# cfframe/spatial-VAE

Measured on AMD Instinct MI355X. Metric: images/sec (ELBO fwd+bwd+step), MNIST 28x28 batch=256, 1/2/4/8 GPU, higher is better.
Workload: dtype f32; 1 GPU; mnist-rotated-translated 28x28 z=2 H=500x2 tanh B=256 (BASELINE configs[1]); global_batch=256, per_gpu_batch=256, pixels=784, parallelism=dp1

## Files before the change

spatial_vae_amd/csrc/api.hip:

```cpp
#include <stdarg.h>
#include <stdio.h>
#include <stdlib.h>
#include <string.h>
#include <math.h>
#include <atomic>
#include <mutex>
#include <iterator>
#include <type_traits>
#include <unordered_map>
#include <vector>

#include "common.h"
#include <hip/hip_ext.h>
#include "dense.h"
#include "wgrad2.h"
#include "elementwise.h"
#include "encoder.h"
#include "split.h"

using namespace svae;

namespace {

thread_local char g_err[512] = "";
// ... 79 lines not shown
    return on;
}

bool split_a0_fragments_only(const Geo& g) {
    static const bool on = [] { const char* e = getenv("SVAE_SPLIT_A0"); return e && e[0] == '1'; }();
    const char* fuse = getenv("SVAE_FUSE_OUT");
    return on && split_mode() && split_l0_on() && split_wgrad_on() && !(fuse && fuse[0] == '1') &&
           (g.act == SVAE_ACT_TANH || g.act == SVAE_ACT_SIGMOID) && g.ntile % 2 == 0 && g.L == 2 && g.in_dim == 2 &&
           !(g.flags & SVAE_FLAG_RESID);
}

int fuse_out_mode() {
    const char* e = getenv("SVAE_FUSE_OUT");
    if (!e) return 2;
    return e[0] == '0' ? 0 : (e[0] == '1' ? 1 : 2);
}
bool split_active(const Geo& g) {
    return split_mode() && (g.act == SVAE_ACT_TANH || g.act == SVAE_ACT_SIGMOID) && g.ntile % 2 == 0;
}
bool rank1_out(const Geo& g) {
    return fuse_out_mode() == 2 && !split_active(g) && g.C == 1 && g.L >= 2 && !(g.flags & SVAE_FLAG_RESID) &&
           (g.act == SVAE_ACT_TANH || g.act == SVAE_ACT_SIGMOID);
}

struct PlanBits {
    unsigned bits;
    unsigned long long seq;
};
std::mutex g_plan_mu;
std::unordered_map<const void*, PlanBits> g_plans;
unsigned long long g_plan_seq = 0;
unsigned plan_bits(const Geo& g) {
    return (rank1_out(g) ? 1u : 0u) | (split_active(g) ? 2u : 0u) | ((unsigned)fuse_out_mode() << 2) |
           (split_a0_fragments_only(g) ? 16u : 0u) | ((split_mode() && split_l0_on()) ? 32u : 0u);
}
void remember_plan(const void* saved, unsigned bits) {
    std::lock_guard<std::mutex> lk(g_plan_mu);
    if (g_plans.size() >= 4096) {
        const unsigned long long cut = g_plan_seq - 2048;
        for (auto it = g_plans.begin(); it != g_plans.end();) it = it->second.seq < cut ? g_plans.erase(it) : std::next(it);
    }
    g_plans[saved] = PlanBits{bits, g_plan_seq++};
}
long recorded_plan(const void* saved) {
    std::lock_guard<std::mutex> lk(g_plan_mu);
    auto it = g_plans.find(saved);
    return it == g_plans.end() ? -1L : (long)it->second.bits;
}

constexpr int kFinishMaxChunks = 64;
int finish_chunks(int N) {
    int c = (N + 1023) / 1024;
    return c < 1 ? 1 : (c > kFinishMaxChunks ? kFinishMaxChunks : c);
}

Plan make_plan(const Geo& g, void* saved, void* ws) {
    Plan p;
    const size_t MH = (size_t)g.Mp * g.Hp;
    Carver cs(saved);
    for (int l = 0; l < g.L; ++l) p.act[l] = cs.take<float>(MH);
    p.savedC = split_mode() ? cs.take<uint4>(MH / 4) : nullptr;
    float* swf[SVAE_MAX_HIDDEN];
    float* swb[SVAE_MAX_HIDDEN];
    for (int l = 0; l + 1 < g.L; ++l) {
        swf[l] = cs.take<float>((size_t)g.Hp * g.Hp);
        swb[l] = cs.take<float>((size_t)g.Hp * g.Hp);
    }
// ... 90 lines not shown
    if ((long)d->B * ((d->N + 31) / 32 * 32) > (1L << 30)) return fail(SVAE_E_INVALID, "B*N too large");
    return SVAE_OK;
}

int check_params(const svae_desc* d, const svae_params* p) {
    if (!p || !p->coord_w || !p->coord_b || !p->out_w || !p->out_b) return fail(SVAE_E_INVALID, "missing parameter pointer");
    if (d->Zd > 0 && !p->latent_w) return fail(SVAE_E_INVALID, "latent_dim > 0 but latent_w is null");
    if ((d->flags & SVAE_FLAG_BILINEAR) && !p->bilinear_w) return fail(SVAE_E_INVALID, "bilinear flag but bilinear_w is null");
    for (int l = 0; l + 1 < d->L; ++l)
        if (!p->hidden_w[l] || !p->hidden_b[l]) return fail(SVAE_E_INVALID, "hidden layer %d parameters are null", l);
    return SVAE_OK;
}

int check_pose(const svae_pose* pose) {
    if (!pose) return fail(SVAE_E_INVALID, "null pose");
    if (!pose->coords && !pose->grid) return fail(SVAE_E_INVALID, "pose needs coords or grid");
    return SVAE_OK;
}

int check_ws(const Plan& p, const void* ws, size_t ws_bytes) {
    if (!ws) return fail(SVAE_E_WORKSPACE, "null workspace");
    if (reinterpret_cast<uintptr_t>(ws) & 255) return fail(SVAE_E_WORKSPACE, "workspace not 256-byte aligned");
    if (ws_bytes < p.ws_bytes) return fail(SVAE_E_WORKSPACE, "workspace too small: %zu < %zu", ws_bytes, p.ws_bytes);
    return SVAE_OK;
}

enum Kind { K_PREPARE = 0, K_LAYER0_FWD, K_DENSE_FWD, K_OUT_FWD, K_DLOGITS, K_OUT_BWD, K_WGRAD, K_WGRAD_REDUCE,
            K_DENSE_DGRAD, K_LAYER0_BWD, K_SMALL_BWD, K_BCE, K_GAUSSIAN, K_LATENT, K_ADAM, K_AUGMENT, K_ENCODER, K_COUNT };
const char* const kKindNames[SVAE_PROF_KINDS] = {"prepare", "layer0_fwd", "dense_fwd", "out_fwd", "dlogits", "out_bwd",
                                                 "wgrad", "wgrad_reduce", "dense_dgrad", "layer0_bwd", "small_bwd", "bce",
                                                 "gaussian", "latent", "adam", "augment", "encoder", "", "", ""};
static_assert(K_COUNT <= SVAE_PROF_KINDS, "svae_profile_read arrays too small");
enum Path { P_DENSE_FP32_FWD = 0, P_DENSE_FP32_DGRAD, P_WGRAD_FP32, P_DENSE_SPLIT_FWD, P_DENSE_SPLIT_DGRAD, P_WGRAD_SPLIT,
            P_OUT_BWD_STREAM, P_OUT_BWD_SPLIT, P_OUT_BWD_RANK1, P_OUT_BWD_FUSED_GENERIC, P_DENSE4, P_DENSE4_TAIL, P_WGRAD2, P_COUNT };
const char* const kPathNames[SVAE_PATH_KINDS] = {"dense_fp32_fwd", "dense_fp32_dgrad", "wgrad_fp32", "dense_split_fwd",
                                                  "dense_split_dgrad", "wgrad_split", "out_bwd_stream", "out_bwd_split",
                                                  "out_bwd_rank1", "out_bwd_fused_generic", "dense4", "dense4_tail", "wgrad2", "", "", ""};
static_assert(P_COUNT <= SVAE_PATH_KINDS, "svae_path_counts array too small");
std::atomic<long long> g_path[SVAE_PATH_KINDS];
inline void took(int path) { g_path[path].fetch_add(1, std::memory_order_relaxed); }

struct ProfRec { hipEvent_t a, b; int kind; };
int g_prof_level = 0;
std::vector<ProfRec> g_prof_used, g_prof_free;

struct Scope;
thread_local Scope* t_attach = nullptr;

struct Scope {
    hipStream_t st;
    ProfRec rec;
    bool on, attach, carried;
    Scope(int kind, hipStream_t s, bool attach_to_launch = false) : st(s), on(false), attach(attach_to_launch), carried(false) {
        std::lock_guard<std::mutex> lk(g_prof_mu);
        if (g_prof_level == 0) return;
        if (g_prof_level == 1 && kind != K_DENSE_FWD && kind != K_DENSE_DGRAD && kind != K_WGRAD) return;
        if (!g_prof_free.empty()) {
            rec = g_prof_free.back();
            g_prof_free.pop_back();
        } else if (hipEventCreate(&rec.a) != hipSuccess || hipEventCreate(&rec.b) != hipSuccess) {
            return;
        }
        rec.kind = kind;
        on = true;
        if (attach) t_attach = this;
        else (void)hipEventRecord(rec.a, st);
    }
    ~Scope() {
        if (!on) return;
        if (attach) t_attach = nullptr;
// ... 253 lines not shown
        if (!cols_ready)
            hipLaunchKernelGGL(split_cols_kernel, dim3(blocks_for(g.noct * g.Hp)), dim3(256), 0, st, dh, pl.splitC[0], g.noct,
                               g.Hp, (const float*)pl.gscale);
        if (!aprev_cols)
            hipLaunchKernelGGL(split_cols_kernel, dim3(blocks_for(g.noct * g.Hp)), dim3(256), 0, st, aprev, pl.splitC[1],
                               g.noct, g.Hp, (const float*)nullptr);
    }
    Scope prof(K_WGRAD, st);
    static bool attr_set = false;
    if (!attr_set) {
        (void)hipFuncSetAttribute(reinterpret_cast<const void*>(&split_wgrad_kernel<true>),
                                  hipFuncAttributeMaxDynamicSharedMemorySize, kSplitWgradLds);
        (void)hipFuncSetAttribute(reinterpret_cast<const void*>(&split_wgrad_kernel<false>),
                                  hipFuncAttributeMaxDynamicSharedMemorySize, kSplitWgradLds);
        attr_set = true;
    }
    SplitWgradArgs w;
    w.dh = pl.splitC[0]; w.ap = aprev_cols ? aprev_cols : pl.splitC[1]; w.slab = pl.slab; w.bslab = pl.bslab; w.gscale = pl.gscale;
    w.nsteps = (long)g.Mp / 16; w.Hp = g.Hp; w.nblk1 = pl.wg_nblk1; w.S = pl.wg_S;
    const dim3 grid(pl.wg_nblk1 * pl.wg_nblk1 * pl.wg_S);
    if (cols_ready) hipLaunchKernelGGL(split_wgrad_kernel<false>, grid, dim3(256), kSplitWgradLds, st, w);
    else hipLaunchKernelGGL(split_wgrad_kernel<true>, grid, dim3(256), kSplitWgradLds, st, w);
}

int use_dense4(const Geo& g, int resid, int lastd) {
    const char* e = getenv("SVAE_DENSE4");
    const int mode = e ? (e[0] == '0' ? 0 : (e[0] == '2' ? 2 : 1)) : 3;
    if (mode == 0 || g.tiles % 4 != 0 || resid || lastd == 1) return 0;
    const bool nt2_ok = g.ntile % 2 == 0;
    if (mode == 2) return nt2_ok ? 2 : 1;
    if (mode == 1) return 1;
    const long wgs2 = ((g.tiles / 4 + 3) / 4) * (g.ntile / 2);
    return (nt2_ok && wgs2 >= 2048) ? 2 : 1;
}

template <int NT, bool DGRAD, bool FIRST, int LASTD, int CF>
void launch_dense4_v(const DenseArgs& a, long groups, long set0, long nsets, hipStream_t st) {
    const dim3 grid((unsigned)(((nsets + 7) / 8) * 8 * ((a.Hp / 32) / NT)));
    constexpr int lds = DenseCfg<NT>::LDS_BYTES + (FIRST ? 4 * 3 * 128 * 4 : 0);
    const long gend = (set0 + nsets) * 4 < groups ? (set0 + nsets) * 4 : groups;
    launch_gemm(dense4_kernel<NT, DGRAD, FIRST, LASTD, CF>, grid, dim3(256), (unsigned)lds, st, a, gend, set0);
}

struct DenseBlocks {
    int nt;
    long m_split;
    int nt_tail;
};

long dense4_main_sets(const Geo& g, long sets, bool tail_ok) {
    const char* e = getenv("SVAE_DENSE4_TAIL");
    if ((e && e[0] == '0') || !tail_ok) return sets;
    if (e && e[0] == '=') {
        const long k = atol(e + 1);
        return (k > 0 && k < sets) ? k : sets;
    }
    static const long slots = [] {
        int dev = 0, cus = 256;
        if (hipGetDevice(&dev) == hipSuccess) (void)hipDeviceGetAttribute(&cus, hipDeviceAttributeMultiprocessorCount, dev);
        return (long)cus * 2;
    }();
    const long nblk = g.ntile / 2;
    const long W = sets * nblk;
    if (slots % nblk != 0) return sets;
    const long full = (W / slots) * slots, rest = W - full;
    if (full < 2 * slots || rest == 0 || W >= 16 * slots || 20 * rest > 9 * slots) return sets;
// ... 193 lines not shown

}

extern "C" {

int svae_abi_version(void) { return SVAE_ABI_VERSION; }
const char* svae_last_error(void) { return g_err; }

size_t svae_saved_bytes(const svae_desc* d) {
    if (check_desc(d) != SVAE_OK) return 0;
    return make_plan(make_geo(*d), nullptr, nullptr).saved_bytes;
}

size_t svae_workspace_bytes(const svae_desc* d) {
    if (check_desc(d) != SVAE_OK) return 0;
    return make_plan(make_geo(*d), nullptr, nullptr).ws_bytes;
}

}

namespace {
int decoder_forward_impl(const svae_desc* d, const svae_params* p, const svae_pose* pose, const float* z, float* y,
                         float* logits, void* saved, void* ws, size_t ws_bytes, svae_stream_t stream, const float* bce_target,
                         float* loglik, float* dll_dy) {
    int rc;
    if ((rc = check_desc(d)) || (rc = check_params(d, p)) || (rc = check_pose(pose))) return rc;
    if (!y) return fail(SVAE_E_INVALID, "y is null");
    if (bce_target && !loglik) return fail(SVAE_E_INVALID, "a Bernoulli target needs the loglik output");
    if (bce_target && (d->flags & SVAE_FLAG_SOFTPLUS))
        return fail(SVAE_E_INVALID, "softplus output with a Bernoulli likelihood: the reference's binary_cross_entropy rejects "
                                    "values above 1 (train_mnist.py:81)");
    if (d->Zd > 0 && !z) return fail(SVAE_E_INVALID, "latent_dim > 0 but z is null");
    if (saved && (reinterpret_cast<uintptr_t>(saved) & 255)) return fail(SVAE_E_WORKSPACE, "saved not 256-byte aligned");
    const Geo g = make_geo(*d);
    Plan pl = make_plan(g, saved, ws);
    if ((rc = check_ws(pl, ws, ws_bytes))) return rc;
    hipStream_t st = static_cast<hipStream_t>(stream);
    const PoseArgs pa = pose_args(pose);
    if (!saved) {
        for (int l = 0; l < g.L; ++l) pl.act[l] = pl.dh[l & 1];
    } else {
        remember_plan(saved, plan_bits(g));
    }

    const char* fuse_e = getenv("SVAE_FUSE_LOGITS");
    const bool fuse_env = !(fuse_e && fuse_e[0] == '0');
    const bool split_fwd = split_mode() && (g.act == SVAE_ACT_TANH || g.act == SVAE_ACT_SIGMOID) && g.ntile % 2 == 0;
    const bool fuse_logits = fuse_env && g.L >= 2 &&
                             (split_fwd ? g.C <= 2
                                        : g.C <= 2 * (use_dense4(g, g.flags & SVAE_FLAG_RESID, 0) ? use_dense4(g, g.flags & SVAE_FLAG_RESID, 0)
                                                                                                   : dense_nt_first(g.ntile)));

    launch_prepare(g, pl, p, pa, z, st);
    const bool split = split_mode() && (g.act == SVAE_ACT_TANH || g.act == SVAE_ACT_SIGMOID) && g.ntile % 2 == 0;
    const bool split_l0 = split_l0_on() && split && g.L >= 2;
    if (split_l0) {
        if (g.act == SVAE_ACT_TANH) launch_layer0_fwd_split<SVAE_ACT_TANH>(g, pl, pa, pl.act[0], saved != nullptr, st);
        else launch_layer0_fwd_split<SVAE_ACT_SIGMOID>(g, pl, pa, pl.act[0], saved != nullptr, st);
    } else {
        switch (g.act) {
            case SVAE_ACT_TANH: launch_layer0_fwd<SVAE_ACT_TANH>(g, pl, pa, pl.act[0], st); break;
            case SVAE_ACT_LEAKYRELU: launch_layer0_fwd<SVAE_ACT_LEAKYRELU>(g, pl, pa, pl.act[0], st); break;
            case SVAE_ACT_RELU: launch_layer0_fwd<SVAE_ACT_RELU>(g, pl, pa, pl.act[0], st); break;
            default: launch_layer0_fwd<SVAE_ACT_SIGMOID>(g, pl, pa, pl.act[0], st); break;
        }
    }
    DenseBlocks cfb{dense_nt_first(g.ntile), (long)g.Mp, 1};
    for (int l = 1; l < g.L; ++l) {
        if (split) {
            launch_split_fwd(g, pl, pl.act[l - 1], p->hidden_w[l - 1], p->hidden_b[l - 1], pl.act[l],
                             (g.flags & SVAE_FLAG_RESID) != 0, (fuse_logits && l == g.L - 1) ? g.C : 0, p->out_w,
                             split_l0 && l == 1, st);
            continue;
        }
        DenseArgs a;
        a.in = pl.act[l - 1];
        a.wp = pl.wf[l - 1];
        a.out = pl.act[l];
        a.bias = p->hidden_b[l - 1];
        a.aux = nullptr;
        a.tiles = g.tiles;
        a.Hp = g.Hp;
        a.H = g.H;
        a.act = g.act;
        a.resid = (g.flags & SVAE_FLAG_RESID) ? 1 : 0;
        a.pose = pa; a.posebuf = nullptr; a.tab = nullptr; a.sgtile = nullptr; a.dfpart = nullptr;
        a.Mp = g.Mp; a.N = g.N; a.Timg = g.Timg;
        a.do_p = nullptr; a.out_w = p->out_w; a.C = g.C;
        a.lpart = pl.dfpart;
        const DenseBlocks used = launch_dense<false>(g, a, st, false, 0, (fuse_logits && l == g.L - 1) ? g.C : 0);
        if (l == g.L - 1) cfb = used;
    }
    if (fuse_logits) {
        Scope prof(K_OUT_FWD, st);
        const int nblk = g.ntile / (split ? split_nt_fwd(g) : cfb.nt);
        const long m_split = split ? (long)g.Mp : cfb.m_split;
        const int nblk_tail = g.ntile / cfb.nt_tail;
        if (bce_target) {
            const int chunks = finish_chunks(g.N);
            hipLaunchKernelGGL(logits_finish_bce_kernel, dim3(g.B, chunks), dim3(g.N > 512 ? 1024 : (g.N > 256 ? 512 : 256)), 0, st,
                               pl.dfpart, p->out_b, bce_target, y, logits, chunks > 1 ? pl.llpart : loglik, dll_dy, row_geo(g), g.C,
                               nblk, (long)g.Mp, m_split, nblk_tail);
            if (chunks > 1)
                hipLaunchKernelGGL(loglik_reduce_kernel, dim3(blocks_for(g.B)), dim3(256), 0, st, pl.llpart, loglik, g.B, chunks);
        }
        else
            hipLaunchKernelGGL(logits_finish_kernel, dim3(blocks_for((long)g.B * g.N)), dim3(256), 0, st, pl.dfpart, p->out_b, y,
                               logits, row_geo(g), g.C, nblk, (g.flags & SVAE_FLAG_SOFTPLUS) ? 1 : 0, (long)g.Mp, m_split, nblk_tail);
        return launch_status("svae_decoder_forward");
    }
    switch (g.C) {
        case 1: launch_out_fwd<1>(g, pl.act[g.L - 1], p, y, logits, st); break;
        case 2: launch_out_fwd<2>(g, pl.act[g.L - 1], p, y, logits, st); break;
        case 3: launch_out_fwd<3>(g, pl.act[g.L - 1], p, y, logits, st); break;
        default: launch_out_fwd<4>(g, pl.act[g.L - 1], p, y, logits, st); break;
    }
    if (bce_target) {
        Scope prof(K_BCE, st);
        hipLaunchKernelGGL(bce_kernel, dim3(g.B), dim3(256), 0, st, y, bce_target, loglik, dll_dy, g.N * g.C);
    }
    return launch_status("svae_decoder_forward");
}
}

extern "C" {

int svae_decoder_forward(const svae_desc* d, const svae_params* p, const svae_pose* pose, const float* z, float* y,
                         float* logits, void* saved, void* ws, size_t ws_bytes, svae_stream_t stream) {
    return decoder_forward_impl(d, p, pose, z, y, logits, saved, ws, ws_bytes, stream, nullptr, nullptr, nullptr);
}

int svae_decoder_forward_bce(const svae_desc* d, const svae_params* p, const svae_pose* pose, const float* z,
                             const float* target, float* y, float* logits, float* loglik, float* dll_dy, void* saved, void* ws,
                             size_t ws_bytes, svae_stream_t stream) {
    if (!target) return fail(SVAE_E_INVALID, "svae_decoder_forward_bce: target is null");
    return decoder_forward_impl(d, p, pose, z, y, logits, saved, ws, ws_bytes, stream, target, loglik, dll_dy);
}

int svae_decoder_backward(const svae_desc* d, const svae_params* p, const svae_pose* pose, const float* z,
                          const float* logits, const float* dy, const float* dy_scale, const void* saved,
                          const svae_grads* grads, float* dz, const svae_pose_grads* pg, void* ws, size_t ws_bytes,
                          svae_stream_t stream) {
    int rc;
    if ((rc = check_desc(d)) || (rc = check_params(d, p)) || (rc = check_pose(pose))) return rc;
    if (!logits || !dy || !saved || !grads) return fail(SVAE_E_INVALID, "logits, dy, saved and grads are required");
    if (d->Zd > 0 && !z) return fail(SVAE_E_INVALID, "latent_dim > 0 but z is null");
    if (reinterpret_cast<uintptr_t>(saved) & 255) return fail(SVAE_E_WORKSPACE, "saved not 256-byte aligned");
    if (pg && (pg->dtheta || pg->ddx) && pose->coords)
        return fail(SVAE_E_INVALID, "dtheta/ddx requested but the pose was given as explicit coords");
    const Geo g = make_geo(*d);
    {
        const long rec = recorded_plan(saved);
        if (rec >= 0 && (unsigned)rec != plan_bits(g))
            return fail(SVAE_E_INVALID, "svae_decoder_backward: `saved` was written by a forward call planned differently (plan "
                        "bits %ld then, %u now): the GEMM mode (svae_gemm_mode_set / SVAE_GEMM) or SVAE_FUSE_OUT changed between "
                        "the forward call and its backward call", rec, plan_bits(g));
    }
    const Plan pl = make_plan(g, const_cast<void*>(saved), ws);
    if ((rc = check_ws(pl, ws, ws_bytes))) return rc;
    hipStream_t st = static_cast<hipStream_t>(stream);
    const PoseArgs pa = pose_args(pose);
    const int resid = (g.flags & SVAE_FLAG_RESID) ? 1 : 0;
    const int fmode = fuse_out_mode();
    const bool split_bwd = split_active(g) && g.L >= 2 && fmode != 1;
    const bool r1 = rank1_out(g);

    {
        Scope prof(K_DLOGITS, st);
        if (split_bwd && hipMemsetAsync(pl.amax, 0, sizeof(unsigned), st) != hipSuccess) return fail(SVAE_E_LAUNCH, "memset failed");
        hipLaunchKernelGGL(dlogits_kernel, dim3(blocks_for((long)g.C * g.Mp)), dim3(256), 0, st, logits, dy, dy_scale,
                           pl.do_p, g.B, g.N, g.Npad, g.C, (g.flags & SVAE_FLAG_SOFTPLUS) ? 1 : 0, (long)g.Mp,
                           split_bwd ? pl.amax : (unsigned*)nullptr);
        if (split_bwd)
            hipLaunchKernelGGL(split_scale_kernel, dim3(1), dim3(256), 0, st, pl.amax, p->out_w, g.C, g.H, pl.gscale);
    }

    int cur = 0;
    const bool fused_out = r1 || (fmode == 1 && g.L >= 2 && !resid && (grads->hidden_w[g.L - 2] || grads->hidden_b[g.L - 2]));
    int ob_nparts = 0;
    static const bool ob_env = [] { const char* e = getenv("SVAE_SPLIT_OB"); return !(e && e[0] == '0'); }();
    const bool split_ob = ob_env && split_bwd && split_wgrad_on() && (grads->hidden_w[g.L - 2] || grads->hidden_b[g.L - 2]);
    if (split_ob) {
        const float* alast = pl.act[g.L - 1];
        float* dh32 = resid ? pl.dh[cur] : nullptr;
        const int nparts = g.act == SVAE_ACT_TANH ? launch_out_bwd_split_a<SVAE_ACT_TANH>(g, pl, alast, p, dh32, st)
                                                  : launch_out_bwd_split_a<SVAE_ACT_SIGMOID>(g, pl, alast, p, dh32, st);
        ob_nparts = nparts;
        Scope prof(K_SMALL_BWD, st);
        hipLaunchKernelGGL(out_bwd_reduce_kernel, dim3(g.C * ((g.Hp + 63) / 64) + 1), dim3(1024), 0, st, pl.wpart, pl.bpart,
// ... 38 lines not shown
                static const bool xcd_grid = [] { const char* e = getenv("SVAE_XCD_GRID"); return !(e && e[0] == '0'); }();
                launch_wgrad(w, pl.wg_S, xcd_grid, last ? g.C : 0, (last && r1) ? (g.act == SVAE_ACT_TANH ? 1 : 2) : 0, st);
            }
            Scope prof(K_WGRAD_REDUCE, st);
            const bool db_elsewhere = split_ob && l == g.L - 1 && split_wgrad_on();
            const WgradReduceArgs ra{pl.slab, pl.bslab, grads->hidden_w[l - 1],
                                     db_elsewhere ? (float*)nullptr : grads->hidden_b[l - 1], g.H, g.Hp, pl.wg_S,
                                     (last && r1) ? p->out_w : (const float*)nullptr};
            if (l == 1 && g.in_dim == 2 && !split_here && tail_merge_on()) {
                tail_r = ra;
                tail_pending = true;
            } else {
                hipLaunchKernelGGL(wgrad_reduce_kernel, dim3((unsigned)(((long)g.H * g.H + 63) / 64)), dim3(256), 0, st, ra);
            }
            if (db_elsewhere && grads->hidden_b[l - 1])
                hipLaunchKernelGGL(colsum_reduce_kernel, dim3(g.Hp / 32), dim3(256), 0, st, pl.hbpart, grads->hidden_b[l - 1],
                                   g.H, g.Hp, ob_nparts);
            if (last)
                hipLaunchKernelGGL(out_bwd_reduce_kernel, dim3(g.C * ((g.Hp + 63) / 64) + 1), dim3(1024), 0, st, pl.wpart, pl.bpart,
                                   grads->out_w, grads->out_b, g.C, g.H, g.Hp, pl.wg_S * 2);
        }
        DenseArgs a;
        a.in = last ? pl.act[l] : pl.dh[cur];
        a.wp = pl.wb[l - 1];
        a.out = pl.dh[cur ^ 1];
        a.bias = nullptr;
        a.aux = pl.act[l - 1];
        a.tiles = g.tiles;
        a.Hp = g.Hp;
        a.H = g.H;
        a.act = g.act;
        a.resid = resid;
        a.pose = pa; a.posebuf = pl.posebuf; a.tab = pl.tab; a.sgtile = pl.sgtile; a.dfpart = pl.dfpart;
        a.Mp = g.Mp; a.N = g.N; a.Timg = g.Timg;
        a.do_p = pl.do_p; a.out_w = p->out_w; a.C = g.C;
        fused_first = (l == 1) && g.in_dim == 2;
        if (split_here)
            launch_split_dgrad(g, pl, pl.dh[cur], p->hidden_w[l - 1], pl.act[l - 1], pl.dh[cur ^ 1], resid != 0, fused_first, pa,
                               split_ob && l == g.L - 1, st);
        else {
            const DenseBlocks used = launch_dense<true>(g, a, st, fused_first, last ? (r1 ? (g.act == SVAE_ACT_TANH ? 2 : 3) : 1) : 0);
            if (l == 1) fb = used;
        }
        cur ^= 1;
    }

    if (tail_pending && !fused_first) {
        tail_pending = false;
        hipLaunchKernelGGL(wgrad_reduce_kernel, dim3((unsigned)(((long)g.H * g.H + 63) / 64)), dim3(256), 0, st, tail_r);
    }
    const bool bil = (g.flags & SVAE_FLAG_BILINEAR) != 0;
    const bool want_coords = pg && (pg->dcoords || pg->dtheta || pg->ddx);
    float* dc = (pg && pg->dcoords) ? pg->dcoords : pl.dcoords;
    {
        Scope prof_l0(K_LAYER0_BWD, st);
        const bool split_first = split_bwd && (g.L == 2 || split_chain_on());
        const bool want_dz = dz && g.Zd > 0;
        if (fused_first) {
            const FirstLayerImageArgs fa{pl.sgtile, split_first ? 2 : 1, g.Timg, g.H, g.Hp, pl.sgimg, p->latent_w,
                                         bil ? p->bilinear_w : nullptr, want_dz ? dz : (float*)nullptr, g.Zd, g.in_dim, pl.dfpart,
                                         g.ntile / (split_first ? split_nt(g) : fb.nt), g.N, g.Npad, (long)g.Mp,
                                         want_coords ? dc : (float*)nullptr, pose->grid, pl.posebuf,
                                         pg ? pg->dtheta : (float*)nullptr, pg ? pg->ddx : (float*)nullptr,
                                         split_first ? (long)g.Mp : fb.m_split, g.ntile / fb.nt_tail};
            const unsigned nimg = (unsigned)g.B * (want_coords ? 2u : 1u);
            if (tail_pending) {
                tail_pending = false;
// ... 301 lines not shown
```

spatial_vae_amd/csrc/common.h:

```cpp
#pragma once
#include <hip/hip_runtime.h>
#include <stdint.h>

#include "../../include/svae.h"

namespace svae {

typedef float f32x16 __attribute__((ext_vector_type(16)));
typedef float v4f __attribute__((ext_vector_type(4)));

constexpr int kSlots = 8;
constexpr int kBiasSlot = 5;

struct Geo {
    int B, N, H, L, Zd, C, in_dim, act, flags;
    int Timg;
    int Npad;
    int Mp;
    int Hp;
    int ntile;
    long noct;
    long tiles;
};

inline Geo make_geo(const svae_desc& d) {
    Geo g;
    g.B = d.B; g.N = d.N; g.H = d.H; g.L = d.L; g.Zd = d.Zd; g.C = d.C;
    g.in_dim = d.in_dim; g.act = d.act; g.flags = d.flags;
    g.Timg = (d.N + 31) / 32;
    g.Npad = g.Timg * 32;
    g.Mp = d.B * g.Npad;
    g.Hp = (d.H + 31) / 32 * 32;
    g.ntile = g.Hp / 32;
    g.noct = (long)g.Mp / 8;
    g.tiles = (long)g.Mp / 32;
    return g;
}

struct PoseArgs {
    const float* coords;
    const float* grid;
    const float* theta;
    const float* dx;
};

__device__ __forceinline__ float fast_rcp(float x) { return __builtin_amdgcn_rcpf(x); }

__device__ __forceinline__ float fast_tanh(float x) {
    float t = __builtin_amdgcn_exp2f(x * 2.885390081777927f);
    return 1.0f - 2.0f * fast_rcp(t + 1.0f);
}
__device__ __forceinline__ float fast_sigmoid(float x) {
    float t = __builtin_amdgcn_exp2f(x * -1.4426950408889634f);
    return fast_rcp(1.0f + t);
}

template <int ACT>
__device__ __forceinline__ float act_fwd(float h) {
    if (ACT == SVAE_ACT_TANH) return fast_tanh(h);
    if (ACT == SVAE_ACT_LEAKYRELU) return h > 0.0f ? h : 0.01f * h;
    if (ACT == SVAE_ACT_RELU) return h > 0.0f ? h : 0.0f;
    return fast_sigmoid(h);
}
template <int ACT>
__device__ __forceinline__ float act_grad(float a) {
    if (ACT == SVAE_ACT_TANH) return 1.0f - a * a;
    if (ACT == SVAE_ACT_LEAKYRELU) return a > 0.0f ? 1.0f : 0.01f;
    if (ACT == SVAE_ACT_RELU) return a > 0.0f ? 1.0f : 0.0f;
    return a * (1.0f - a);
// ... 121 lines not shown
```

spatial_vae_amd/csrc/dense.h:

```cpp
#pragma once
#include "common.h"

namespace svae {

struct DenseArgs {
    const float* in;
    const float* wp;
    float* out;
    const float* bias;
    const float* aux;
    long tiles;
    int Hp;
    int H;
    int act;
    int resid;
    PoseArgs pose;
    const float4* posebuf;
    const float* tab;
    float* sgtile;
    float* dfpart;
    long Mp;
    int N, Timg;
    const float* do_p;
    const float* out_w;
    int C;
    float* lpart;
};

template <int ACT, bool DGRAD>
__device__ __forceinline__ float4 dense_epilogue(float4 v, float bias, float4 aux) {
    if (DGRAD) {
        v.x *= act_grad<ACT>(aux.x); v.y *= act_grad<ACT>(aux.y);
        v.z *= act_grad<ACT>(aux.z); v.w *= act_grad<ACT>(aux.w);
    } else {
        v.x = act_fwd<ACT>(v.x + bias); v.y = act_fwd<ACT>(v.y + bias);
        v.z = act_fwd<ACT>(v.z + bias); v.w = act_fwd<ACT>(v.w + bias);
    }
    return v;
}

__device__ __forceinline__ void glds16(const float* gsrc, unsigned lds_byte_addr) {
    unsigned keep;
    asm volatile(
        "s_mov_b32 %0, m0\n\ts_mov_b32 m0, %2\n\ts_nop 0\n\tglobal_load_lds_dwordx4 %1, off\n\ts_mov_b32 m0, %0"
        : "=&s"(keep)
        : "v"(gsrc), "s"(lds_byte_addr)
        : "memory");
}
__device__ __forceinline__ void dma_wait_all() { asm volatile("s_waitcnt vmcnt(0)" ::: "memory"); }
__device__ __forceinline__ void glds16_s(const void* sbase, unsigned voff, unsigned lds_byte_addr) {
    unsigned keep;
    asm volatile(
        "s_mov_b32 %0, m0\n\ts_mov_b32 m0, %3\n\ts_nop 0\n\tglobal_load_lds_dwordx4 %1, %2\n\ts_mov_b32 m0, %0"
        : "=&s"(keep)
        : "v"(voff), "s"(sbase), "s"(lds_byte_addr)
// ... 743 lines not shown
```

spatial_vae_amd/csrc/dense4.h:

```cpp
#pragma once
#include "dense.h"

namespace svae {

typedef float f32x4v __attribute__((ext_vector_type(4)));
typedef float f32x2v __attribute__((ext_vector_type(2)));

template <int OFF>
__device__ __forceinline__ void load_a4(const float* p, f32x4v& v) {
    asm volatile("global_load_dwordx4 %0, %1, off offset:%2" : "+v"(v) : "v"(p), "i"(OFF) : "memory");
}
template <int N>
__device__ __forceinline__ void wait_vm4(f32x4v& v) {
    asm volatile("s_waitcnt vmcnt(%1)" : "+v"(v) : "i"(N) : "memory");
}
template <int LASTD>
__device__ __forceinline__ f32x4v rank1_actgrad(f32x4v x) {
    f32x4v r;
#pragma unroll
    for (int i = 0; i < 4; ++i) r[i] = __builtin_fmaf(-x[i], x[i], LASTD == 2 ? 1.0f : x[i]);
    return r;
}

template <int NT>
struct Dense4Occ {
    static constexpr int value = NT == 1 ? 3 : 2;
};

template <int NT, bool DGRAD, bool FIRST, int LASTD, int CF>
__device__ __forceinline__ void dense4_body(const DenseArgs& a, long groups, long set0, unsigned bid) {
    static_assert(NT == 1 || NT == 2, "4 NT accumulator tiles: two waves per SIMD up to NT = 2");
    static_assert(!FIRST || DGRAD, "FIRST is a data-gradient epilogue");
    static_assert(LASTD == 0 || ((LASTD == 2 || LASTD == 3) && DGRAD), "LASTD: the rank-1 data-gradient forms only");
    static_assert(CF == 0 || (!DGRAD && CF <= SVAE_MAX_OUT), "CF = output channels of the forward epilogue's W_o contraction");
    extern __shared__ __attribute__((aligned(16))) float smem[];
    using Cfg = DenseCfg<NT>;
    constexpr int NB = Cfg::NB, G = Cfg::G, CHUNK = Cfg::CHUNK, NINSTR = Cfg::NINSTR;
    const int lane = threadIdx.x & 63;
    const int wave = __builtin_amdgcn_readfirstlane(threadIdx.x >> 6);
    const int nl = lane & 31, h = lane >> 5;
    const int Hp = a.Hp;
    const int noct = Hp / 8;
    const int nchunk = noct / G;
    const int ntile = Hp / 32;
    const int nblk = ntile / NT;
    const long local = bid >> 3;
    const int nb = (int)(local % nblk);
    const long set = set0 + (local / nblk) * 8 + (bid & 7);
    const long rg = set * 4 + wave;
    const bool live = rg < groups;
    const long rgl = live ? rg : groups - 1;

    const float* arow = a.in + ((rgl * 16 + (nl >> 1)) * (long)Hp + 4 * h) * 8 + (nl & 1) * 4;
    const float* bfrag = smem + lane * 4;
    const unsigned lds_base = (unsigned)(size_t)(__attribute__((address_space(3))) float*)smem;

    f32x16 acc[4][NT];
#pragma unroll
    for (int c = 0; c < 4; ++c)
#pragma unroll
        for (int t = 0; t < NT; ++t)
#pragma unroll
            for (int r = 0; r < 16; ++r) acc[c][t][r] = 0.0f;

    constexpr int PW = (NINSTR + 3) / 4;
    unsigned poff[PW], pm0[PW];
#pragma unroll
    for (int j = 0; j < PW; ++j) {
        const int idx = wave + 4 * j;
        const int gl = (idx < NINSTR ? idx : NINSTR - 1) / NT, tt = (idx < NINSTR ? idx : NINSTR - 1) % NT;
        poff[j] = (unsigned)(((gl * ntile + nb * NT + tt) * 256 + lane * 4) * 4);
        pm0[j] = lds_base + (unsigned)(idx < NINSTR ? idx : NINSTR - 1) * 1024u;
    }
    const unsigned chunk_bytes = (unsigned)(G * ntile) * 1024u;
    auto stage_piece = [&](int c, int buf, int j) {
        glds16_s(reinterpret_cast<const char*>(a.wp) + (long)c * chunk_bytes, poff[j], pm0[j] + (unsigned)(buf * CHUNK) * 4u);
    };
    auto stage = [&](int c, int buf) {
#pragma unroll
        for (int j = 0; j < PW; ++j) stage_piece(c, buf, j);
    };
    auto read_b = [&](int o, float4 (&b)[NT]) {
        const float* base = bfrag + ((o / G) & 1) * CHUNK + (o % G) * NT * 256;
#pragma unroll
        for (int t = 0; t < NT; ++t) b[t] = *reinterpret_cast<const float4*>(base + t * 256);
    };
    constexpr int P = PW;
    constexpr int PE = (P + 3) / 4;
    static_assert(G == 4, "the slot offsets assume 4 octets per chunk");

    float* rowx = smem + 2 * CHUNK + wave * (3 * 128);
    if (FIRST) {
#pragma unroll
        for (int rr = 0; rr < 2; ++rr) {
            const int row = lane + 64 * rr;
            const long tile = rgl * 4 + (row >> 5);
            const int b = (int)(tile / a.Timg);
            const int i = (int)(tile % a.Timg) * 32 + (row & 31);
            const float4 pb = a.posebuf[b];
            const float* cbase = a.pose.coords ? a.pose.coords + (long)b * a.N * 2 : a.pose.grid;
            const float2 g2 = *reinterpret_cast<const float2*>(cbase + (long)(i < a.N ? i : a.N - 1) * 2);
            const bool in = i < a.N;
            rowx[row] = in ? pb.x * g2.x - pb.y * g2.y + pb.z : 0.0f;
            rowx[128 + row] = in ? pb.y * g2.x + pb.x * g2.y + pb.w : 0.0f;
            if (LASTD != 0) rowx[256 + row] = a.do_p[rgl * 128 + row];
        }
    }
    stage(0, 0);
    stage(nchunk > 1 ? 1 : 0, 1);
    f32x4v av[G][4];
    float4 b0[NT], b1[NT];
#pragma unroll
    for (int gl = 0; gl < G; ++gl)
#pragma unroll
        for (int e = 0; e < 4; ++e) av[gl][e] = f32x4v{0.0f, 0.0f, 0.0f, 0.0f};
    load_a4<0>(arow, av[0][0]); load_a4<32>(arow, av[0][1]); load_a4<64>(arow, av[0][2]); load_a4<96>(arow, av[0][3]);
    load_a4<256>(arow, av[1][0]); load_a4<288>(arow, av[1][1]); load_a4<320>(arow, av[1][2]); load_a4<352>(arow, av[1][3]);
    load_a4<512>(arow, av[2][0]); load_a4<544>(arow, av[2][1]); load_a4<576>(arow, av[2][2]); load_a4<608>(arow, av[2][3]);
    load_a4<768>(arow, av[3][0]); load_a4<800>(arow, av[3][1]); load_a4<832>(arow, av[3][2]); load_a4<864>(arow, av[3][3]);
#pragma unroll
    for (int gl = 0; gl < G; ++gl)
#pragma unroll
        for (int e = 0; e < 4; ++e) wait_vm4<0>(av[gl][e]);
    __syncthreads();
    read_b(0, b0);
    const int spare = nchunk & 1;
    auto kstep = [&](const f32x4v& x, const float4 (&bf)[NT], int e) {
#pragma unroll
        for (int t = 0; t < NT; ++t) {
            const float bv = e == 0 ? bf[t].x : e == 1 ? bf[t].y : e == 2 ? bf[t].z : bf[t].w;
            acc[0][t] = __builtin_amdgcn_mfma_f32_32x32x2f32(x[0], bv, acc[0][t], 0, 0, 0);
// ... 142 lines not shown
                            lp[c][4 * r + 2] += v.z * wo[c][t]; lp[c][4 * r + 3] += v.w * wo[c][t];
                        }
                    }
                }
                if (CF > 0 && t == NT - 1) {
#pragma unroll
                    for (int c = 0; c < CFN; ++c) {
                        float s4[4];
                        half_reduce16(lp[c], s4);
                        if (nl < 4) {
                            const int cls = ((nl & 1) << 1) | (nl >> 1);
                            *reinterpret_cast<float4*>(a.lpart + ((long)nb * CFN + c) * a.Mp + rgl * 128 + 32 * q + 16 * h + 4 * cls) =
                                make_float4(s4[0], s4[1], s4[2], s4[3]);
                        }
                    }
                }
            }
        } else {
            float4 xa[2][NT][2];
            auto fetch_aux = [&](int hp, float4 (&fa)[NT][2]) {
                const int q = hp >> 1, rh = hp & 1;
#pragma unroll
                for (int t = 0; t < NT; ++t)
#pragma unroll
                    for (int r2 = 0; r2 < 2; ++r2) fa[t][r2] = *reinterpret_cast<const float4*>(a.aux + voff(q, 2 * rh + r2, t));
            };
            fetch_aux(0, xa[0]);
            float2 w[NT];
            float sv[NT], g0[NT], g1[NT];
#pragma unroll
            for (int hp = 0; hp < 8; ++hp) {
                const int q = hp >> 1, rh = hp & 1;
                const long tile = rgl * 4 + q;
                if (rh == 0) {
                    const int b = (int)(tile / a.Timg);
#pragma unroll
                    for (int t = 0; t < NT; ++t) {
                        w[t] = *reinterpret_cast<const float2*>(a.tab + ((long)b * Hp + nb * NB + t * 32 + nl) * kSlots);
                        sv[t] = 0.0f; g0[t] = 0.0f; g1[t] = 0.0f;
                    }
                }
                if (hp + 1 < 8) fetch_aux(hp + 1, xa[(hp + 1) & 1]);
                const float* rx = rowx + 32 * q + 16 * h + 8 * rh;
                float4 x0v[2], x1v[2], dq[2];
#pragma unroll
                for (int r2 = 0; r2 < 2; ++r2) {
                    x0v[r2] = *reinterpret_cast<const float4*>(rx + 4 * r2);
                    x1v[r2] = *reinterpret_cast<const float4*>(rx + 128 + 4 * r2);
                    if (LASTD != 0) dq[r2] = *reinterpret_cast<const float4*>(rx + 256 + 4 * r2);
                }
                float pd[16];
#pragma unroll
                for (int j = 0; j < 16; ++j) pd[j] = 0.0f;
#pragma unroll
                for (int t = 0; t < NT; ++t)
#pragma unroll
                    for (int r2 = 0; r2 < 2; ++r2) {
                        const float4 v = value(q, 2 * rh + r2, t, xa[hp & 1][t][r2], dq[r2]);
                        const float vv[4] = {v.x, v.y, v.z, v.w};
                        const float xx0[4] = {x0v[r2].x, x0v[r2].y, x0v[r2].z, x0v[r2].w};
                        const float xx1[4] = {x1v[r2].x, x1v[r2].y, x1v[r2].z, x1v[r2].w};
#pragma unroll
                        for (int cc = 0; cc < 4; ++cc) {
                            const int j = 4 * r2 + cc;
                            sv[t] += vv[cc];
                            g0[t] += vv[cc] * xx0[cc];
                            g1[t] += vv[cc] * xx1[cc];
                            pd[j] += vv[cc] * w[t].x;
                            pd[8 + j] += vv[cc] * w[t].y;
                        }
                    }
                float s4[4];
                half_reduce16(pd, s4);
                if (nl < 4) {
                    const int cls = ((nl & 1) << 1) | (nl >> 1);
                    float* dst = a.dfpart + ((long)nb * a.Mp + tile * 32 + 16 * h + 8 * rh + 4 * (cls & 1)) * 2 + (cls >> 1);
                    dst[0] = s4[0]; dst[2] = s4[1]; dst[4] = s4[2]; dst[6] = s4[3];
                }
                if (rh == 1) {
#pragma unroll
                    for (int t = 0; t < NT; ++t) {
                        const float G0 = g0[t] + __shfl_xor(g0[t], 32), G1 = g1[t] + __shfl_xor(g1[t], 32);
                        const float S = sv[t] + __shfl_xor(sv[t], 32);
                        const int k = nb * NB + t * 32 + nl;
                        if (h == 0) *reinterpret_cast<float4*>(a.sgtile + (tile * (long)Hp + k) * 4) = make_float4(G0, G1, S, 0.0f);
                    }
                }
            }
        }
    };
    switch (a.act) {
        case SVAE_ACT_TANH: epi(std::integral_constant<int, SVAE_ACT_TANH>()); break;
        case SVAE_ACT_LEAKYRELU: epi(std::integral_constant<int, SVAE_ACT_LEAKYRELU>()); break;
        case SVAE_ACT_RELU: epi(std::integral_constant<int, SVAE_ACT_RELU>()); break;
        default: epi(std::integral_constant<int, SVAE_ACT_SIGMOID>()); break;
    }
}

template <int NT, bool DGRAD, bool FIRST, int LASTD, int CF>
__global__ __launch_bounds__(256, Dense4Occ<NT>::value) void dense4_kernel(DenseArgs a, long groups, long set0) {
    dense4_body<NT, DGRAD, FIRST, LASTD, CF>(a, groups, set0, blockIdx.x);
}

template <bool DGRAD, bool FIRST, int LASTD, int CF>
__global__ __launch_bounds__(256, 2) void dense4_dual_kernel(DenseArgs a, long groups, long sets_main, unsigned grid_main) {
    if (blockIdx.x < grid_main) {
        const long gmain = sets_main * 4 < groups ? sets_main * 4 : groups;
        dense4_body<2, DGRAD, FIRST, LASTD, CF>(a, gmain, 0, blockIdx.x);
    } else {
        dense4_body<1, DGRAD, FIRST, LASTD, CF>(a, groups, sets_main, blockIdx.x - grid_main);
    }
}

}
```

Baseline: 96730 images/s.

## Pad pixel rows to a 16-row granule instead of 32 in dense4 path

Adds an optional 16-row padding granule for per-image pixel rows when it lowers padding (784 pads to 784 instead of 800) and the dense4 path is in use. Geometry, pose row indexing and the per-tile reduction slot mapping are rewritten to handle 32-row tiles that straddle two images, and the plan bits record the granule so that forward and backward stay consistent. The goal is to cut wasted padded rows in the GEMMs and elementwise work. It adds index arithmetic, extra partial-sum writes for straddling tiles, and an early exit for out-of-range sets.

```diff
diff --git a/spatial_vae_amd/csrc/api.hip b/spatial_vae_amd/csrc/api.hip
--- a/spatial_vae_amd/csrc/api.hip
+++ b/spatial_vae_amd/csrc/api.hip
@@ -135,7 +135,7 @@
 unsigned long long g_plan_seq = 0;
 unsigned plan_bits(const Geo& g) {
     return (rank1_out(g) ? 1u : 0u) | (split_active(g) ? 2u : 0u) | ((unsigned)fuse_out_mode() << 2) |
-           (split_a0_fragments_only(g) ? 16u : 0u) | ((split_mode() && split_l0_on()) ? 32u : 0u);
+           (split_a0_fragments_only(g) ? 16u : 0u) | ((split_mode() && split_l0_on()) ? 32u : 0u) | (g.g16 ? 64u : 0u);
 }
 void remember_plan(const void* saved, unsigned bits) {
     std::lock_guard<std::mutex> lk(g_plan_mu);
@@ -292,10 +292,12 @@
                                                  "gaussian", "latent", "adam", "augment", "encoder", "", "", ""};
 static_assert(K_COUNT <= SVAE_PROF_KINDS, "svae_profile_read arrays too small");
 enum Path { P_DENSE_FP32_FWD = 0, P_DENSE_FP32_DGRAD, P_WGRAD_FP32, P_DENSE_SPLIT_FWD, P_DENSE_SPLIT_DGRAD, P_WGRAD_SPLIT,
-            P_OUT_BWD_STREAM, P_OUT_BWD_SPLIT, P_OUT_BWD_RANK1, P_OUT_BWD_FUSED_GENERIC, P_DENSE4, P_DENSE4_TAIL, P_WGRAD2, P_COUNT };
+            P_OUT_BWD_STREAM, P_OUT_BWD_SPLIT, P_OUT_BWD_RANK1, P_OUT_BWD_FUSED_GENERIC, P_DENSE4, P_DENSE4_TAIL, P_WGRAD2,
+            P_GRANULE16, P_COUNT };
 const char* const kPathNames[SVAE_PATH_KINDS] = {"dense_fp32_fwd", "dense_fp32_dgrad", "wgrad_fp32", "dense_split_fwd",
                                                   "dense_split_dgrad", "wgrad_split", "out_bwd_stream", "out_bwd_split",
-                                                  "out_bwd_rank1", "out_bwd_fused_generic", "dense4", "dense4_tail", "wgrad2", "", "", ""};
+                                                  "out_bwd_rank1", "out_bwd_fused_generic", "dense4", "dense4_tail", "wgrad2", "granule16",
+                                                  "", ""};
 static_assert(P_COUNT <= SVAE_PATH_KINDS, "svae_path_counts array too small");
 std::atomic<long long> g_path[SVAE_PATH_KINDS];
 inline void took(int path) { g_path[path].fetch_add(1, std::memory_order_relaxed); }
@@ -615,6 +617,15 @@
     if (mode == 1) return 1;
     const long wgs2 = ((g.tiles / 4 + 3) / 4) * (g.ntile / 2);
     return (nt2_ok && wgs2 >= 2048) ? 2 : 1;
+}
+
+bool granule16_ok(const svae_desc& d) {
+    const char* e = getenv("SVAE_GRANULE");
+    if (e && e[0] == '3') return false;
+    const int n16 = (d.N + 15) / 16 * 16;
+    if (n16 == (d.N + 31) / 32 * 32 || ((long)d.B * n16) % 128 != 0) return false;
+    if (d.L < 2 || split_mode() || (d.flags & SVAE_FLAG_RESID) || fuse_out_mode() == 1) return false;
+    return use_dense4(make_geo(d, true), 0, 0) != 0;
 }
 
 template <int NT, bool DGRAD, bool FIRST, int LASTD, int CF>
@@ -874,7 +885,8 @@
                                     "values above 1 (train_mnist.py:81)");
     if (d->Zd > 0 && !z) return fail(SVAE_E_INVALID, "latent_dim > 0 but z is null");
     if (saved && (reinterpret_cast<uintptr_t>(saved) & 255)) return fail(SVAE_E_WORKSPACE, "saved not 256-byte aligned");
-    const Geo g = make_geo(*d);
+    const Geo g = make_geo(*d, granule16_ok(*d));
+    if (g.g16) took(P_GRANULE16);
     Plan pl = make_plan(g, saved, ws);
     if ((rc = check_ws(pl, ws, ws_bytes))) return rc;
     hipStream_t st = static_cast<hipStream_t>(stream);
@@ -927,7 +939,7 @@
         a.act = g.act;
         a.resid = (g.flags & SVAE_FLAG_RESID) ? 1 : 0;
         a.pose = pa; a.posebuf = nullptr; a.tab = nullptr; a.sgtile = nullptr; a.dfpart = nullptr;
-        a.Mp = g.Mp; a.N = g.N; a.Timg = g.Timg;
+        a.Mp = g.Mp; a.N = g.N; a.Timg = g.Timg; a.Npad = g.Npad;
         a.do_p = nullptr; a.out_w = p->out_w; a.C = g.C;
         a.lpart = pl.dfpart;
         const DenseBlocks used = launch_dense<false>(g, a, st, false, 0, (fuse_logits && l == g.L - 1) ? g.C : 0);
@@ -990,13 +1002,14 @@
     if (reinterpret_cast<uintptr_t>(saved) & 255) return fail(SVAE_E_WORKSPACE, "saved not 256-byte aligned");
     if (pg && (pg->dtheta || pg->ddx) && pose->coords)
         return fail(SVAE_E_INVALID, "dtheta/ddx requested but the pose was given as explicit coords");
-    const Geo g = make_geo(*d);
+    const Geo g = make_geo(*d, granule16_ok(*d));
+    if (g.g16) took(P_GRANULE16);
     {
         const long rec = recorded_plan(saved);
         if (rec >= 0 && (unsigned)rec != plan_bits(g))
             return fail(SVAE_E_INVALID, "svae_decoder_backward: `saved` was written by a forward call planned differently (plan "
-                        "bits %ld then, %u now): the GEMM mode (svae_gemm_mode_set / SVAE_GEMM) or SVAE_FUSE_OUT changed between "
-                        "the forward call and its backward call", rec, plan_bits(g));
+                        "bits %ld then, %u now): the GEMM mode (svae_gemm_mode_set / SVAE_GEMM), SVAE_FUSE_OUT or the row granule "
+                        "(SVAE_DENSE4, SVAE_GRANULE) changed between the forward call and its backward call", rec, plan_bits(g));
     }
     const Plan pl = make_plan(g, const_cast<void*>(saved), ws);
     if ((rc = check_ws(pl, ws, ws_bytes))) return rc;
@@ -1101,7 +1114,7 @@
         a.act = g.act;
         a.resid = resid;
         a.pose = pa; a.posebuf = pl.posebuf; a.tab = pl.tab; a.sgtile = pl.sgtile; a.dfpart = pl.dfpart;
-        a.Mp = g.Mp; a.N = g.N; a.Timg = g.Timg;
+        a.Mp = g.Mp; a.N = g.N; a.Timg = g.Timg; a.Npad = g.Npad;
         a.do_p = pl.do_p; a.out_w = p->out_w; a.C = g.C;
         fused_first = (l == 1) && g.in_dim == 2;
         if (split_here)
diff --git a/spatial_vae_amd/csrc/common.h b/spatial_vae_amd/csrc/common.h
--- a/spatial_vae_amd/csrc/common.h
+++ b/spatial_vae_amd/csrc/common.h
@@ -16,6 +16,7 @@
     int B, N, H, L, Zd, C, in_dim, act, flags;
     int Timg;
     int Npad;
+    int g16;
     int Mp;
     int Hp;
     int ntile;
@@ -23,18 +24,25 @@
     long tiles;
 };
 
-inline Geo make_geo(const svae_desc& d) {
+inline Geo make_geo(const svae_desc& d, bool granule16 = false) {
     Geo g;
     g.B = d.B; g.N = d.N; g.H = d.H; g.L = d.L; g.Zd = d.Zd; g.C = d.C;
     g.in_dim = d.in_dim; g.act = d.act; g.flags = d.flags;
     g.Timg = (d.N + 31) / 32;
-    g.Npad = g.Timg * 32;
+    g.g16 = granule16 ? 1 : 0;
+    g.Npad = granule16 ? (d.N + 15) / 16 * 16 : g.Timg * 32;
     g.Mp = d.B * g.Npad;
     g.Hp = (d.H + 31) / 32 * 32;
     g.ntile = g.Hp / 32;
     g.noct = (long)g.Mp / 8;
     g.tiles = (long)g.Mp / 32;
     return g;
+}
+
+__host__ __device__ __forceinline__ long tile_slot(long m0, int Npad, int Timg) {
+    const long b = m0 / Npad;
+    const long j = (m0 - b * Npad) >> 4;
+    return b * Timg + ((j + ((b * (Npad >> 4)) & 1)) >> 1);
 }
 
 struct PoseArgs {
diff --git a/spatial_vae_amd/csrc/dense.h b/spatial_vae_amd/csrc/dense.h
--- a/spatial_vae_amd/csrc/dense.h
+++ b/spatial_vae_amd/csrc/dense.h
@@ -21,6 +21,7 @@
     float* dfpart;
     long Mp;
     int N, Timg;
+    int Npad;
     const float* do_p;
     const float* out_w;
     int C;
diff --git a/spatial_vae_amd/csrc/dense4.h b/spatial_vae_amd/csrc/dense4.h
--- a/spatial_vae_amd/csrc/dense4.h
+++ b/spatial_vae_amd/csrc/dense4.h
@@ -47,6 +47,7 @@
     const long local = bid >> 3;
     const int nb = (int)(local % nblk);
     const long set = set0 + (local / nblk) * 8 + (bid & 7);
+    if (set * 4 >= groups) return;
     const long rg = set * 4 + wave;
     const bool live = rg < groups;
     const long rgl = live ? rg : groups - 1;
@@ -94,9 +95,9 @@
 #pragma unroll
         for (int rr = 0; rr < 2; ++rr) {
             const int row = lane + 64 * rr;
-            const long tile = rgl * 4 + (row >> 5);
-            const int b = (int)(tile / a.Timg);
-            const int i = (int)(tile % a.Timg) * 32 + (row & 31);
+            const long m = rgl * 128 + row;
+            const int b = (int)(m / a.Npad);
+            const int i = (int)(m - (long)b * a.Npad);
             const float4 pb = a.posebuf[b];
             const float* cbase = a.pose.coords ? a.pose.coords + (long)b * a.N * 2 : a.pose.grid;
             const float2 g2 = *reinterpret_cast<const float2*>(cbase + (long)(i < a.N ? i : a.N - 1) * 2);
@@ -305,8 +306,10 @@
             for (int hp = 0; hp < 8; ++hp) {
                 const int q = hp >> 1, rh = hp & 1;
                 const long tile = rgl * 4 + q;
+                const long m0 = tile * 32 + 16 * h;
+                const int b = (int)(m0 / a.Npad);
+                const bool straddle = (tile * 32) / a.Npad != (tile * 32 + 16) / a.Npad;
                 if (rh == 0) {
-                    const int b = (int)(tile / a.Timg);
 #pragma unroll
                     for (int t = 0; t < NT; ++t) {
                         w[t] = *reinterpret_cast<const float2*>(a.tab + ((long)b * Hp + nb * NB + t * 32 + nl) * kSlots);
@@ -351,12 +354,15 @@
                     dst[0] = s4[0]; dst[2] = s4[1]; dst[4] = s4[2]; dst[6] = s4[3];
                 }
                 if (rh == 1) {
+                    const long slot = tile_slot(m0, a.Npad, a.Timg);
 #pragma unroll
                     for (int t = 0; t < NT; ++t) {
                         const float G0 = g0[t] + __shfl_xor(g0[t], 32), G1 = g1[t] + __shfl_xor(g1[t], 32);
                         const float S = sv[t] + __shfl_xor(sv[t], 32);
                         const int k = nb * NB + t * 32 + nl;
-                        if (h == 0) *reinterpret_cast<float4*>(a.sgtile + (tile * (long)Hp + k) * 4) = make_float4(G0, G1, S, 0.0f);
+                        if (straddle || h == 0)
+                            *reinterpret_cast<float4*>(a.sgtile + (slot * Hp + k) * 4) =
+                                straddle ? make_float4(g0[t], g1[t], sv[t], 0.0f) : make_float4(G0, G1, S, 0.0f);
                     }
                 }
             }
```

Result: no change. 97270 images/s (median of 6 runs) (+0.5%).
